# aaron-randreth/modulation-mfcc

Hardware: AMD Instinct MI355X
Metric: MFCC+mod-spectrum frames/sec (higher is better)
Workload: dtype f32; 1 GPU; BASELINE configs[2] per GPU: 1024 clips x 10 s x 16000 Hz, win 400 hop 160 n_fft 512, 40 mel (fmax 8000), 13 MFCC + modulation spectrum (rFFT 1024 over trajectories); frames_per_clip=1001, clips_total=1024, parallelism=clips sharded x1, hsa_ipc_mode_legacy=0, settle_calls=744, full=False, fused_tail=True

## Files before the change

### include/modmfcc.h

```cpp
#ifndef MODMFCC_H
#define MODMFCC_H

#include <stddef.h>
#include <stdint.h>

#ifdef __cplusplus
extern "C" {
#endif

#define MM_VERSION 123

typedef enum mm_status {
  MM_OK = 0,
  MM_ERR_INVALID_ARG = -1,
  MM_ERR_UNSUPPORTED = -2,
  MM_ERR_HIP = -3,
  MM_ERR_WORKSPACE = -4,
  MM_ERR_ALLOC = -5
} mm_status;

typedef struct mm_config {
  double sr;
  int32_t n_fft;
  int32_t win_length;
// ... 26 lines not shown
const char* mm_strerror(int status);
const char* mm_last_hip_error(void);

int mm_config_default(mm_config* cfg);
int mm_config_validate(const mm_config* cfg);
int64_t mm_num_frames(const mm_config* cfg, int64_t n_samples);
int32_t mm_num_bins(const mm_config* cfg);
int32_t mm_mod_fft_len(const mm_config* cfg, int64_t n_frames);
int mm_build_window(const mm_config* cfg, float* out );
int mm_build_mel(const mm_config* cfg, float* out );
int mm_build_dct(const mm_config* cfg, float* out );
int mm_build_mel_sweep(const mm_config* cfg, int n_waves, float* wlo ,
                       float* whi , int32_t* d , int32_t* part );
int mm_build_mel_runs(const mm_config* cfg, int n_waves, int32_t* hdr, int32_t hdr_cap, float* grp,
                      int32_t grp_cap, int32_t* part, int32_t* counts);
int mm_build_butter_sos(int order, double wn, double* sos );

int mm_plan_create(const mm_config* cfg, mm_plan** out);
int mm_plan_destroy(mm_plan* plan);
int mm_plan_config(const mm_plan* plan, mm_config* out);
int mm_plan_kernel_path(const mm_plan* plan);
int mm_plan_fused_dct(const mm_plan* plan);
int mm_plan_set_fuse_dct(mm_plan* plan, int on);
int mm_plan_fused_tail(const mm_plan* plan, int64_t batch, int64_t n_samples);
int mm_plan_set_fuse_tail(mm_plan* plan, int on);
int mm_plan_force_generic(mm_plan* plan, int on);
int mm_plan_set_variant(mm_plan* plan, int variant);
size_t mm_workspace_bytes(const mm_plan* plan, int64_t batch, int64_t n_samples);

int mm_mfcc_f32(mm_plan* plan, const float* d_audio, int64_t batch, int64_t n_samples,
                int64_t audio_stride, float* d_mfcc, void* d_workspace, size_t ws_bytes,
                void* stream);

int mm_logmel_f32(mm_plan* plan, const float* d_audio, int64_t batch, int64_t n_samples,
                  int64_t audio_stride, float* d_logmel, float* d_clipmax, void* stream);

int mm_stft_power_f32(mm_plan* plan, const float* d_audio, int64_t batch, int64_t n_samples,
                      int64_t audio_stride, float* d_power, void* stream);

int mm_rfft_f32(mm_plan* plan, const float* d_in, int64_t rows, int64_t in_len,
// ... 151 lines not shown
```

### modulation_mfcc_amd/_lib.py

```python
from __future__ import annotations

import ctypes as C
import os

_HERE = os.path.dirname(os.path.abspath(__file__))
LIB_PATH = os.environ.get("MODMFCC_LIB") or os.path.join(_HERE, "libmodmfcc.so")

MM_OK = 0
MM_ERR_INVALID_ARG = -1
MM_ERR_UNSUPPORTED = -2
MM_ERR_HIP = -3
MM_ERR_WORKSPACE = -4
MM_ERR_ALLOC = -5

STAGES = ("logmel", "dct", "modspec", "rfft", "power", "change", "init", "reserved")
MM_NUM_STAGES = 8


class mm_config(C.Structure):
    _fields_ = [
        ("sr", C.c_double),
        ("n_fft", C.c_int32),
        ("win_length", C.c_int32),
        ("hop_length", C.c_int32),
# ... 73 lines not shown

PROTOTYPES = {
    "mm_version": (C.c_int, []),
    "mm_strerror": (C.c_char_p, [C.c_int]),
    "mm_last_hip_error": (C.c_char_p, []),
    "mm_config_default": (C.c_int, [_cfgp]),
    "mm_config_validate": (C.c_int, [_cfgp]),
    "mm_num_frames": (_i64, [_cfgp, _i64]),
    "mm_num_bins": (C.c_int32, [_cfgp]),
    "mm_mod_fft_len": (C.c_int32, [_cfgp, _i64]),
    "mm_build_window": (C.c_int, [_cfgp, _vp]),
    "mm_build_mel": (C.c_int, [_cfgp, _vp]),
    "mm_build_dct": (C.c_int, [_cfgp, _vp]),
    "mm_build_mel_sweep": (C.c_int, [_cfgp, C.c_int, _vp, _vp, _vp, _vp]),
    "mm_build_mel_runs": (C.c_int, [_cfgp, C.c_int, _vp, C.c_int32, _vp, C.c_int32, _vp, _vp]),
    "mm_build_butter_sos": (C.c_int, [C.c_int, C.c_double, _vp]),
    "mm_plan_create": (C.c_int, [_cfgp, C.POINTER(_vp)]),
    "mm_plan_destroy": (C.c_int, [_vp]),
    "mm_plan_config": (C.c_int, [_vp, _cfgp]),
    "mm_plan_kernel_path": (C.c_int, [_vp]),
    "mm_plan_fused_dct": (C.c_int, [_vp]),
    "mm_plan_set_fuse_dct": (C.c_int, [_vp, C.c_int]),
    "mm_plan_fused_tail": (C.c_int, [_vp, _i64, _i64]),
    "mm_plan_set_fuse_tail": (C.c_int, [_vp, C.c_int]),
    "mm_mfcc_modspec_f32": (C.c_int, [_vp, _vp, _i64, _i64, _i64, _vp, _vp, _vp, C.c_size_t, _vp]),
    "mm_plan_force_generic": (C.c_int, [_vp, C.c_int]),
    "mm_plan_set_variant": (C.c_int, [_vp, C.c_int]),
    "mm_workspace_bytes": (C.c_size_t, [_vp, _i64, _i64]),
    "mm_mfcc_f32": (C.c_int, [_vp, _vp, _i64, _i64, _i64, _vp, _vp, C.c_size_t, _vp]),
    "mm_logmel_f32": (C.c_int, [_vp, _vp, _i64, _i64, _i64, _vp, _vp, _vp]),
    "mm_stft_power_f32": (C.c_int, [_vp, _vp, _i64, _i64, _i64, _vp, _vp]),
    "mm_rfft_f32": (C.c_int, [_vp, _vp, _i64, _i64, _i64, C.c_int32, _vp, _vp]),
    "mm_modspec_f32": (C.c_int, [_vp, _vp, _i64, _i64, _vp, _vp]),
    "mm_mfcc_change_f64": (C.c_int, [_vp, _vp, _i64, _i64, C.c_int32, C.c_int32, _vp, C.c_int32, _vp,
                                     C.c_int32, _vp, _vp, C.c_size_t, _vp]),
    "mm_sosfiltfilt_f64": (C.c_int, [_vp, _i64, _i64, _i64, _vp, C.c_int32, _vp, _vp, C.c_size_t, _vp]),
    "mm_sosfiltfilt_workspace_bytes": (C.c_size_t, [_i64, _i64]),
    "mm_sosfiltfilt_f32_f64": (C.c_int, [_vp, _i64, _i64, _i64, _vp, C.c_int32, _vp, _vp, C.c_size_t, _vp]),
    "mm_stencil_f64": (C.c_int, [C.POINTER(mm_stencil), _vp, _i64, _i64, _i64, _vp, _vp]),
# ... 75 lines not shown
```

### modulation_mfcc_amd/csrc/mm_api.hip

```cpp
#include <memory>
#include <utility>

#include "mm_common.h"
#include "mm_plan.h"

thread_local std::string g_hip_err;

struct StftParams {
  const float* audio;
  int64_t batch, n_samples, stride, n_frames;
  int n_fft, log2nc, hop, n_bins, n_mels;
  float preemph, amin, db_offset;
  const float* window;
  const float2* tw;
  const int* mel_start;
  const int* mel_len;
  const int* mel_off;
  const float* mel_w;
  float* out_power;
  float* out_logmel;
  int* clip_key;
  int frames_per_wave;
};

// ... 240 lines not shown
}
int mm_build_mel_sweep(const mm_config* c, int n_waves, float* wlo, float* whi, int32_t* d, int32_t* part) {
  int s = mm::validate(c);
  if (s) return s;
  if (n_waves < 1 || !wlo || !whi || !d || !part) return MM_ERR_INVALID_ARG;
  std::vector<float> mel((size_t)c->n_mels * (c->n_fft / 2 + 1));
  mm::build_mel(*c, mel.data());
  mm::MelSweep sw;
  if (!mm::build_mel_sweep(*c, mel.data(), n_waves, &sw)) return MM_ERR_UNSUPPORTED;
  std::memcpy(wlo, sw.wlo.data(), sw.wlo.size() * 4);
  std::memcpy(whi, sw.whi.data(), sw.whi.size() * 4);
  std::memcpy(d, sw.d.data(), sw.d.size() * 4);
  std::memcpy(part, sw.part.data(), sw.part.size() * 4);
  return MM_OK;
}
int mm_build_mel_runs(const mm_config* c, int n_waves, int32_t* hdr, int32_t hdr_cap, float* grp,
                      int32_t grp_cap, int32_t* part, int32_t* counts) {
  int s = mm::validate(c);
  if (s) return s;
  if (n_waves < 1 || !hdr || !grp || !part || !counts) return MM_ERR_INVALID_ARG;
  std::vector<float> mel((size_t)c->n_mels * (c->n_fft / 2 + 1));
  mm::build_mel(*c, mel.data());
  mm::MelSweep sw;
  if (!mm::build_mel_sweep(*c, mel.data(), n_waves, &sw)) return MM_ERR_UNSUPPORTED;
  mm::MelRuns r;
  mm::build_mel_runs(*c, sw, n_waves, &r);
  counts[0] = (int32_t)(r.hdr.size() / 4);
  counts[1] = (int32_t)(r.grp.size() / 8);
  if (counts[0] > hdr_cap || counts[1] > grp_cap) return MM_ERR_WORKSPACE;
  std::memcpy(hdr, r.hdr.data(), r.hdr.size() * 4);
  std::memcpy(grp, r.grp.data(), r.grp.size() * 4);
  std::memcpy(part, r.part.data(), r.part.size() * 4);
  return MM_OK;
}
int mm_build_butter_sos(int order, double wn, double* sos) { return mm::build_butter_sos(order, wn, sos); }


static std::vector<float> packed_run_table(const mm::MelRuns& r) {
  std::vector<float> tab(r.hdr.size() + r.grp.size());
  std::memcpy(tab.data(), r.hdr.data(), r.hdr.size() * 4);
  std::memcpy(tab.data() + r.hdr.size(), r.grp.data(), r.grp.size() * 4);
  for (size_t g = 0; g < r.grp.size() / 8; ++g) {
    float* q = tab.data() + r.hdr.size() + 8 * g;
    const float t[8] = {q[0], q[4], q[1], q[5], q[2], q[6], q[3], q[7]};
    std::memcpy(q, t, sizeof t);
  }
  return tab;
}
// ... 279 lines not shown
    const double wts_d[16] = {1, 1, 1, MM_S16F_W, 1, 1, 1, MM_S16F_W, 1, 1, 1, MM_S16F_W, 1, 1, 1, MM_S16F_W};
    double extra[16];
    for (int w = 0; w < 16; ++w) extra[w] = (!single && wts_d[w] < 1.0) ? 700.0 : 0.0;
    mm::MelSweep swf;
    if (!mm::build_mel_sweep(c, h.melp, 16, &swf, single ? nullptr : wts_d)) return;
    mm::MelRuns rf;
    mm::build_mel_runs(c, swf, 16, &rf);
    if (ef.skip)
      for (size_t r = 0; r < rf.hdr.size() / 4; ++r) {
        const int d = rf.hdr[4 * r + 3];
        if (d >= 0 && d < c.n_mels && ef.empty[d]) rf.hdr[4 * r + 0] |= 1 << 16;
      }
    const std::vector<float> tab = packed_run_table(rf);
    std::vector<int> wave_of_part;
    const std::vector<int> part = balance_parts_over_simds(rf, extra, &wave_of_part);
    unsigned long long roles = ~0ull;
    for (int f = 0; f < 4; ++f) {
      const int w = single ? f : wave_of_part[4 * f + 3];
      roles = (roles & ~(0xFull << (4 * w))) | ((unsigned long long)f << (4 * w));
    }
    const size_t tab_end = (size_t)MM_S16_TAB_OFF(p->s16.nr, xa) + tab.size() * 4;
    const unsigned lt_off = (unsigned)align_up(tab_end, 16);
    const unsigned dcta_off = lt_off + (single ? 1u : 2u) * (unsigned)lt_rows * 320u;
    const unsigned red_off = (unsigned)align_up((size_t)dcta_off + dcta.size() * 4, 16);
    const size_t lds = (size_t)red_off + 2 * 16 * 8;
    if (lds > MM_LM_LDS_MAX) continue;
    mm_plan::S16F& f = p->s16f;
    f.ok = p->upload(&f.d_tab, tab.data(), tab.size() * 4) == MM_OK &&
           p->upload(&f.d_part, part.data(), part.size() * 4) == MM_OK &&
           p->upload(&f.d_dcta, dcta.data(), dcta.size() * 4) == MM_OK;
    if (!f.ok) return;
    f.n_runs = (int)(rf.hdr.size() / 4); f.n_tab16 = (int)(tab.size() / 4);
    f.lt_rows = lt_rows; f.nk = nk; f.kb = kbn; f.roles = roles;
    f.flags = (single ? MM_S16F_SINGLE : 0) | (ef.skip ? MM_S16F_SKIP : 0);
    f.lt_off = lt_off; f.dcta_off = dcta_off; f.red_off = red_off; f.lds_bytes = lds;
    if (!xa && p->s16.xa) {
      p->s16.xa = false;
      p->s16.lds_bytes = (size_t)MM_S16_TAB_OFF(p->s16.nr, false) + tab16_bytes;
    }
    return;
  }
}

static void setup_m12(mm_plan* p, const PlanHost& h) {
  const mm_config& c = p->cfg;
  mm_plan::M12& m = p->m12;
  M12Tables mt;
  const int s_floats = (47 * c.hop_length + 512 + 255) & ~255;
  const int nr = (s_floats / 256 + 15) / 16;
  if (nr > 3 || !build_m12_tables(*h.ce, h.melp, h.dct.data(), &mt)) return;
// ... 273 lines not shown
}

int mm_plan_set_fuse_dct(mm_plan* p, int on) {
  if (!p) return MM_ERR_INVALID_ARG;
  const int prev = !p->user.no_fuse;
  p->user.no_fuse = on ? 0 : 1;
  return prev;
}

int mm_plan_set_fuse_tail(mm_plan* p, int on) {
  if (!p) return MM_ERR_INVALID_ARG;
  const int prev = p->user.no_fuse_tail ? 0 : (p->user.fuse_tail_wide ? 2 : 1);
  p->user.no_fuse_tail = on ? 0 : 1;
  p->user.fuse_tail_wide = on == 2 ? 1 : 0;
  return prev;
}

int mm_plan_set_variant(mm_plan* p, int variant) {
  if (!p || variant < 0 || variant > MM_K_H16 || variant == MM_K_ANY) return MM_ERR_INVALID_ARG;
  const int prev = p->user.variant;
  p->user.variant = variant;
  return prev;
}

int mm_plan_force_generic(mm_plan* p, int on) {
  if (!p) return MM_ERR_INVALID_ARG;
  int prev = p->user.force_generic;
  p->user.force_generic = on ? 1 : 0;
  return prev;
}
// ... 151 lines not shown
  if (q.n_tiles > 0x7FFFFFFF) return MM_ERR_INVALID_ARG;
  int64_t grid = q.n_tiles < p->num_cus ? q.n_tiles : p->num_cus;
  if (d.kernel == MM_K_W8) {
    hipLaunchKernelGGL(mode == 0 ? logmel512_kernel<0> : logmel512_kernel<1>, dim3((unsigned)grid), dim3(512), p->w8.lds_bytes, st, q);
    return MM_OK;
  }
  q.mel_tab = (const float4*)p->w16.d_tab; q.n_runs = p->w16.n_runs; q.n_tab16 = p->w16.n_tab16;
  q.wave_part = p->w16.d_part;
  if (d.kernel == MM_K_W16) {
    hipLaunchKernelGGL(mode == 0 ? logmel512w_kernel<0> : logmel512w_kernel<1>, dim3((unsigned)grid), dim3(1024), p->w16.lds_bytes, st, q);
    return MM_OK;
  }
  size_t lds = p->s16.lds_bytes;
  if (d.fused_dct) {
    const mm_plan::S16F& f = p->s16f;
    q.mel_tab = (const float4*)f.d_tab; q.n_runs = f.n_runs; q.n_tab16 = f.n_tab16;
    q.wave_part = f.d_part;
    q.out_mfcc = o.mfcc; q.key_nmin = o.key_nmin; q.dct_a = f.d_dcta; q.n_mfcc = p->cfg.n_mfcc;
    q.dct_nk = f.nk; q.dct_kb = f.kb; q.lt_rows = f.lt_rows;
    q.lt_off = f.lt_off; q.dcta_off = f.dcta_off; q.dct_roles = f.roles;
    q.dct_flags = f.flags | (p->s16.halfwin ? MM_S16F_HALFWIN : 0);
    q.lt_b2 = (f.flags & MM_S16F_SINGLE) ? 0 : f.lt_rows;
    if (p->cfg.top_db < 0.0f) q.out_logmel = nullptr;
    lds = f.lds_bytes;
    q.red_off = f.red_off;
    if (d.clip) {
      q.out_mod = (float2*)o.mod; q.n_mod = o.mod ? c.n_mod : 0; q.dct_t = p->base.d_dct_t; q.dct_kp = p->kp; q.top_db = p->cfg.top_db;
      grid = c.batch < p->num_cus ? c.batch : p->num_cus;
      const size_t per = (size_t)((c.batch + grid - 1) / grid);
      lds = std::max((size_t)f.red_off + per * 128, (size_t)MM_S16_FIN_TAB_OFF + MM_S16_FIN_TAB_BYTES);
      lds = std::max(lds, (size_t)MM_S16_DELTA_OFF((size_t)f.red_off, per, q.n_mod) + per * 4);
      if (q.n_mod == 2048) {
        q.tw = (const float2*)p->rf2k.d_lane_tab;
        lds = std::max(lds, (size_t)MM_S16_FIN2K_BYTES);
      }
      mode = 2;
// ... 258 lines not shown
```

### modulation_mfcc_amd/csrc/mm_fft16.hip.inc

```
#pragma once

namespace f16 {

__device__ __forceinline__ constexpr int P16(int k) { return 4 * (k & 3) + (k >> 2); }

__device__ __forceinline__ float2 cmulf(float2 a, float2 w) {
  return make_float2(fmaf(-a.y, w.y, a.x * w.x), fmaf(a.y, w.x, a.x * w.y));
}

__device__ __forceinline__ void radix4(float2& v0, float2& v1, float2& v2, float2& v3) {
  const float2 t0 = make_float2(v0.x + v2.x, v0.y + v2.y);
  const float2 t1 = make_float2(v0.x - v2.x, v0.y - v2.y);
  const float2 t2 = make_float2(v1.x + v3.x, v1.y + v3.y);
  const float2 t3 = make_float2(v1.x - v3.x, v1.y - v3.y);
  v0 = make_float2(t0.x + t2.x, t0.y + t2.y);
  v2 = make_float2(t0.x - t2.x, t0.y - t2.y);
  v1 = make_float2(t1.x + t3.y, t1.y - t3.x);
  v3 = make_float2(t1.x - t3.y, t1.y + t3.x);
}

__device__ __forceinline__ void dft16(float2 (&x)[16]) {
#pragma unroll
  for (int b = 0; b < 4; ++b) radix4(x[b], x[4 + b], x[8 + b], x[12 + b]);
  const float C1 = 0.92387953251128674f, S1 = 0.38268343236508977f, H = 0.70710678118654752f;
// ... 277 lines not shown
  const float* dct_a;
  int n_mfcc, dct_nk, dct_kb, lt_rows;
  int lt_b2;
  unsigned lt_off, dcta_off;
  unsigned long long dct_roles;
  int dct_flags;
  float2* out_mod;
  const float* dct_t;
  int n_mod, dct_kp;
  float top_db;
  unsigned red_off;
};

#define MM_S16F_SINGLE 1
#define MM_S16F_SKIP 2
#define MM_S16F_HALFWIN 8
#define MM_LM_PITCH 260
#define MM_LM_P_FLOATS (64 * MM_LM_PITCH)
#define MM_LM_EX_OFF (MM_LM_P_FLOATS * 4)
#define MM_LM_WIN_OFF (MM_LM_EX_OFF + 8 * f16::Geo<1>::WAVE_C * 8)
#define MM_LM_TAB_OFF (MM_LM_WIN_OFF + 512 * 4)

#include "mm_tile512.hip.inc"

struct LmItem {
  const float* a;
  int64_t t_first;
  bool live;
  bool interior;
};
// ... 143 lines not shown
```

### modulation_mfcc_amd/csrc/mm_internal.h

```cpp
#ifndef MM_INTERNAL_H
#define MM_INTERNAL_H

#include <vector>

#include "../../include/modmfcc.h"

namespace mm {

struct MelCsr {
  std::vector<int> start, len, off;
  std::vector<float> w;
};

struct MelSweep {
  std::vector<float> wlo, whi;
  std::vector<int> d;
  std::vector<int> part;
};
bool build_mel_sweep(const mm_config& c, const float* dense, int n_waves, MelSweep* out, const double* weights = nullptr);

struct MelRuns {
  std::vector<int> hdr;
  std::vector<float> grp;
  std::vector<int> part;
};
void build_mel_runs(const mm_config& c, const MelSweep& sw, int n_waves, MelRuns* out);

int validate(const mm_config* c);
void build_window(const mm_config& c, float* out);
void build_mel(const mm_config& c, float* out);
void build_dct(const mm_config& c, float* out);
void build_twiddles(int n, float* out);
int build_butter_sos(int order, double wn, double* sos);
void build_mel_csr(const mm_config& c, const float* dense, MelCsr* csr);

}
#endif
```

### modulation_mfcc_amd/csrc/mm_logmel16s.hip.inc

```
#pragma once

struct S16Fin {
  const float* logmel;
  float* mfcc;
  float2* mod;
  const float2* tw;
  const float* dct_t;
  int n_frames, n_mels, n_mfcc, dct_kp, n_mod;
  float top_db;
  float L0;
  const float* dct_e;
};

template <int R>
__device__ __forceinline__ void s16_fin_fill_tab(const float2* tw_generic, MM_LDS mm_v2f* tab) {
  typedef f16::Geo<R> G;
  const MM_GLOBAL mm_v2f* tw = (const MM_GLOBAL mm_v2f*)tw_generic;
  for (int idx = threadIdx.x; idx < G::LPR * MM_S16_FIN_REC + 15; idx += 1024) {
    mm_v2f v;
    if (idx < G::LPR * MM_S16_FIN_REC) {
      const int q = idx / MM_S16_FIN_REC, e = idx - q * MM_S16_FIN_REC;
      if (e < 15) {
        v = tw[(q * (e + 1)) * (MM_TW_N / G::NC)];
      } else {
// ... 383 lines not shown
  float* P = reinterpret_cast<float*>(smem);
  float* S = reinterpret_cast<float*>(smem + MM_S16_S_OFF(XA));
  const int lane = threadIdx.x & 63;
  const int wave = __builtin_amdgcn_readfirstlane(threadIdx.x >> 6);
  const int q = lane & 15, row = lane >> 4;
  const float* lt = reinterpret_cast<const float*>(smem + MM_S16_LT_OFF(NR, XA)) + q * MM_W16_LT_PITCH;

  for (int i = threadIdx.x; i < 16 * MM_W16_LT_PITCH; i += 1024)
    reinterpret_cast<float*>(smem + MM_S16_LT_OFF(NR, XA))[i] = p.lane_tab[i];
  if (threadIdx.x < 64 * 3) P[(threadIdx.x / 3) * MM_S16_PITCH(XA) + 257 + threadIdx.x % 3] = 0.0f;

  for (int i = threadIdx.x; i < p.n_tab16; i += 1024)
    reinterpret_cast<float4*>(smem + MM_S16_TAB_OFF(NR, XA))[i] = p.mel_tab[i];
  const int run0 = p.wave_part[wave * 4 + 0], run1 = p.wave_part[wave * 4 + 1];
  const int m0 = p.wave_part[wave * 4 + 2];
  const bool fused = MODE == 2 || (MODE == 1 && p.out_mfcc != nullptr);
  float* Lt = reinterpret_cast<float*>(smem + p.lt_off);
  const int role = fused ? (int)((p.dct_roles >> (4 * wave)) & 15) : 15;
  const bool lt_single = fused && p.lt_b2 == 0;
  const bool halfwin = NR <= 2 && (p.dct_flags & MM_S16F_HALFWIN) != 0;
  if (fused) {
    for (int i = threadIdx.x; i < (p.lt_b2 + p.lt_rows) * 80; i += 1024) Lt[i] = 0.0f;
    for (int i = threadIdx.x; i < p.dct_kb * p.dct_nk * 64 + 16 * p.dct_kb; i += 1024)
      reinterpret_cast<float*>(smem + p.dcta_off)[i] = p.dct_a[i];
  }
  float vmin = INFINITY;
  int pb = 0, pt0 = 0;
  bool has_prev = false;
  auto dct_tile = [&](const float* Lp, int cb, int ct0) {
    int ln = lane;
// ... 156 lines not shown
        v.z = (ok && s0 + 2 < n) ? v.z : 0.0f; v.w = (ok && s0 + 3 < n) ? v.w : 0.0f;
      } else {
        v.x = ok ? v.x : 0.0f; v.y = ok ? v.y : 0.0f; v.z = ok ? v.z : 0.0f; v.w = ok ? v.w : 0.0f;
      }
      reinterpret_cast<float4*>(S)[threadIdx.x + 1024 * j] = v;
    }
  };
  if (tile_begin < tile_end) {
    stage_load(b, tl);
    stage_store(tl);
  }
  __syncthreads();
  float2 wp[8];
  tile512_read_wp(wp, lt);

  MM_STAMP_BEGIN(16)
  for (int tile = tile_begin; tile < tile_end; ++tile) {
    const int t0 = tl * 64;
    MM_STAMP_AT(9)
    if (++ntl == tpc) { ntl = 0; ++nb; }
    const bool more = tile + 1 < tile_end;
    stage_load(more ? nb : b, more ? ntl : tl);
    MM_STAMP_AT(11)
    if (t0 + 4 * wave < (int)p.n_frames) {
    float2 x[16];
    if (halfwin) {
      if (hop_odd) {
#pragma unroll
        for (int n1 = 4; n1 < 12; ++n1) x[n1] = make_float2(sxf[32 * n1], sxf[32 * n1 + 1]);
      } else {
#pragma unroll
        for (int n1 = 4; n1 < 12; ++n1) x[n1] = sx[16 * n1];
      }
      const float4* w4 = reinterpret_cast<const float4*>(lt) + 2;
// ... 125 lines not shown
    if (MODE == 0) {
      tile512_store_power_tile(p.out_power, P, MM_S16_PITCH(XA), b, t0, p.n_frames, wave, 16, lane);
    } else {
      const bool valid = (t0 + lane) < p.n_frames;
      float* o = p.out_logmel + ((int64_t)b * p.n_mels + m0) * p.n_frames + t0 + lane;
      const float* pl = P + lane * MM_S16_PITCH(XA);
      const float4* hdr = reinterpret_cast<const float4*>(smem + MM_S16_TAB_OFF(NR, XA));
      const float4* grp = hdr + p.n_runs;
      float carry = 0.0f;
      if (run0 < run1) {
        float4 h = hdr[run0];
        for (int r = run0; r < run1; ++r) {
          const int k4e = __builtin_amdgcn_readfirstlane(__float_as_int(h.x));
          const int k4 = k4e & 0xFFFF;
          const bool empty_d = (k4e >> 16) & 1;
          const int ng = __builtin_amdgcn_readfirstlane(__float_as_int(h.y));
          const int go = __builtin_amdgcn_readfirstlane(__float_as_int(h.z));
          const int dd = __builtin_amdgcn_readfirstlane(__float_as_int(h.w));
          if (r + 1 < run1) h = hdr[r + 1];
          const float4* pp = reinterpret_cast<const float4*>(pl + k4);
          const MM_LDS mm_v4f* gw = (const MM_LDS mm_v4f*)(grp + 2 * go);
          asm volatile("" : "+v"(gw));
          float sa = 0.0f, sb = 0.0f;
          MM_STAMP_AT(12)
#pragma unroll 2
          for (int g = 0; g < ng; ++g) {
            const float4 pv = pp[g];
            const mm_v4f wa = gw[2 * g], wb = gw[2 * g + 1];
            sa = fmaf(wa.x, pv.x, sa); sb = fmaf(wa.y, pv.x, sb);
            sa = fmaf(wa.z, pv.y, sa); sb = fmaf(wa.w, pv.y, sb);
            sa = fmaf(wb.x, pv.z, sa); sb = fmaf(wb.y, pv.z, sb);
            sa = fmaf(wb.z, pv.w, sa); sb = fmaf(wb.w, pv.w, sb);
          }
          MM_STAMP_AT(13)
          float dbm = __builtin_nanf("");
          if (dd >= m0) {
            if (!empty_d) {
              const float v = carry + sa;
              const float db = 3.0102999566398120f * __builtin_amdgcn_logf(mm_max_raw_s(v, p.amin)) - p.db_offset;
              if (valid && p.out_logmel) *o = db;
              dbm = valid ? db : dbm;
              if (fused) Lt[((tile & 1) * p.lt_b2 + dd) * 80 + lane] = db;
            }
            o += p.n_frames;
          }
          mm_max_acc(vmax, dbm);
          mm_min_acc(vmin, dbm);
          carry = sb;
          MM_STAMP_AT(14)
        }
      }
      const bool clip_done = (tile + 1 == tile_end) || (ntl == 0);
      if (clip_done) {
        vmax = wave_max(vmax);
        if (p.key_nmin || clip_mode) vmin = wave_min(vmin);
        if (clip_mode) {
          if (lane == 0)
            reinterpret_cast<float2*>(smem + p.red_off)[(b - tile_begin / tpc) * 16 + wave] = make_float2(vmax, vmin);
        } else if (lane == 0 && vmax > -INFINITY) {
          atomicMax(p.clip_key + b, float_key(vmax));
          if (p.key_nmin) atomicMax(p.key_nmin + b, float_key(-vmin));
        }
        vmax = -INFINITY; vmin = INFINITY;
      }
    }
    MM_STAMP_AT(7)
    wg_barrier_lds();
    MM_STAMP_AT(8)
    pb = b; pt0 = t0; has_prev = true;
    b = nb; tl = ntl;
  }
  if (role < 4 && has_prev) dct_tile(Lt + (((tile_end - 1) & 1) * p.lt_b2) * 80, pb, pt0);
  if (clip_mode && has_prev) {
    S16Fin f;
    f.logmel = p.out_logmel; f.mfcc = p.out_mfcc; f.mod = p.out_mod; f.tw = p.tw; f.dct_t = p.dct_t;
    f.n_frames = (int)p.n_frames; f.n_mels = p.n_mels; f.n_mfcc = p.n_mfcc; f.dct_kp = p.dct_kp; f.n_mod = p.n_mod;
    f.top_db = p.top_db;
    f.dct_e = (p.dct_flags & MM_S16F_SKIP) ? p.dct_a + p.dct_kb * p.dct_nk * 64 : nullptr;
    f.L0 = mm_empty_level(p.amin, p.db_offset);
    s16_finalize_all(f, tile_begin / tpc, (tile_end - tile_begin) / tpc, p.red_off,
                     (int)((p.batch + gridDim.x - 1) / gridDim.x));
  }
  MM_STAMP_END(16)
}

// ... 34 lines not shown
```

### modulation_mfcc_amd/csrc/mm_plan.h

```cpp
#pragma once
#include "mm_common.h"

struct AnyPlan {
  int nn = 0, packed = 0, n_pass = 0, radix[16] = {0}, M = 0, log2M = 0, tpf = 64;
  unsigned grp_bytes = 0, b_off = 0, p_off = 0;
  float2 *d_tw = nullptr, *d_split = nullptr, *d_chirp = nullptr, *d_bhat = nullptr;
  float* d_tabpack = nullptr;
  int tab_floats = 0, o_tw = 0, o_split = 0, o_chirp = 0, o_melw = 0, o_mstart = 0, o_mlen = 0, o_moff = 0;
  bool lds_tab = false;
  bool ok = false;
  int fb = 0;
  int reg2 = 0, reg2_r2 = 0;
  unsigned fb_grp_bytes = 0;
};

#define MM_M12_MW 4
#define MM_M12_UMAX 12

#define MM_MAX_TIMED 16384
#define MM_MAX_SAMPLES (((int64_t)1 << 29) - 8192)

struct mm_plan {
  mm_config cfg{};
  int device = 0;
// ... 20 lines not shown
    int n_pairs = 0, n_tab16 = 0; size_t lds_bytes = 0;
  } h16;
  struct S16 {
    int nr = 0;
    bool xa = false;
    bool halfwin = false;
    size_t lds_bytes = 0;
  } s16;
  struct S16F {
    bool ok = false;
    float *d_tab = nullptr, *d_dcta = nullptr; int* d_part = nullptr;
    int n_runs = 0, n_tab16 = 0, lt_rows = 0, nk = 0, kb = 0;
    int flags = 0;
    unsigned lt_off = 0, dcta_off = 0, red_off = 0;
    unsigned long long roles = 0; size_t lds_bytes = 0;
  } s16f;
  struct M12 {
    bool ok = false, fused_dct = false;
    float *d_a = nullptr, *d_dct = nullptr, *d_zeros = nullptr;
    int units[MM_M12_MW * MM_M12_UMAX * 4] = {}, n_units[8] = {};
    int nb = 0, nr = 0, s_floats = 0, n_a2 = 0;
    unsigned win_off = 0, tw_off = 0, a_off = 0, dct_off = 0, part_off = 0, cnt_off = 0;
    size_t lds_bytes = 0;
  } m12;
  struct Wpf {
    bool ok = false; float *d_lane_tab = nullptr, *d_mel_lane = nullptr;
    int r = 0, waves = 0, group_max = 0; size_t lds_bytes = 0;
    bool w16 = false; size_t lds16 = 0;
    bool half = false; int pairs = 0;
    int waves_half = 0; size_t lds_half = 0;
// ... 1 lines not shown
  } wpf;
  struct DctFm {
    float* d_a = nullptr;
    float* d_wave_a = nullptr;
    int kb = 0, wave_nk = 0, ch = 0;
  } dctfm;
  struct Rf2k { bool ok = false; float* d_lane_tab = nullptr; } rf2k;
  AnyPlan any;

  struct Switches {
    int variant = 0;
    int force_generic = 0;
    int no_fuse = 0;
    int no_fuse_tail = 0;
    int fuse_tail_wide = 0;
  } user;
  struct Timing {
    int on = 0, ev_used = 0;
    std::vector<hipEvent_t> ev_pool;
    std::vector<int> ev_stage;
    double t_sum[MM_NUM_STAGES] = {};
    int64_t t_cnt[MM_NUM_STAGES] = {};
  } timing;

  mm_plan() = default;
  mm_plan(const mm_plan&) = delete; mm_plan& operator=(const mm_plan&) = delete;
  ~mm_plan() { for (void* d : owned) (void)hipFree(d); }
  template <class T>
  int upload(T** dst, const void* src, size_t bytes) {
    HIP_TRY(hipMalloc((void**)dst, bytes));
// ... 37 lines not shown
```

### modulation_mfcc_amd/csrc/mm_tables.cpp

```cpp
#include "mm_internal.h"

#include <algorithm>
#include <cmath>
#include <complex>
#include <cstring>
#include <vector>

namespace mm {

static const double kPi = 3.14159265358979323846;

int validate(const mm_config* c) {
  if (!c) return MM_ERR_INVALID_ARG;
  if (!(c->sr > 0.0)) return MM_ERR_INVALID_ARG;
  if (c->n_fft < 2) return MM_ERR_INVALID_ARG;
  if (c->n_fft > 8192) return MM_ERR_UNSUPPORTED;
  if (c->win_length < 1 || c->win_length > c->n_fft) return MM_ERR_INVALID_ARG;
  if (c->hop_length < 1) return MM_ERR_INVALID_ARG;
  if (c->n_mels < 1 || c->n_mels > 256) return MM_ERR_INVALID_ARG;
  if (c->n_mfcc < 1 || c->n_mfcc > c->n_mels) return MM_ERR_INVALID_ARG;
  if (!(c->fmin >= 0.0) || !(c->fmax > c->fmin)) return MM_ERR_INVALID_ARG;
  if (!(c->amin > 0.0f)) return MM_ERR_INVALID_ARG;
  if (c->center != 1) return MM_ERR_UNSUPPORTED;
  if (c->n_mod_fft != 0 &&
// ... 221 lines not shown
      const int left_waves = n_waves - 1 - w;
      if (n_mels - m1 < left_waves) m1 = std::max(m0, n_mels - left_waves);
    }
    int kb, ke;
    range_of(m0, m1, &kb, &ke);
    if (m1 <= m0) { kb = 0; ke = 0; }
    out->part[w * 4 + 0] = kb;
    out->part[w * 4 + 1] = ke;
    out->part[w * 4 + 2] = m0;
    out->part[w * 4 + 3] = m1;
    m = m1;
  }
  return true;
}

void build_mel_runs(const mm_config& c, const MelSweep& sw, int n_waves, MelRuns* out) {
  const int n_bins = c.n_fft / 2 + 1;
  out->hdr.clear(); out->grp.clear();
  out->part.assign((size_t)n_waves * 4, 0);
  for (int w = 0; w < n_waves; ++w) {
    const int m0 = sw.part[w * 4 + 2], m1 = sw.part[w * 4 + 3];
    out->part[w * 4 + 0] = (int)(out->hdr.size() / 4);
    out->part[w * 4 + 2] = m0;
    out->part[w * 4 + 3] = m1;
    if (m1 > m0) {
      for (int d = m0 - 1; d <= m1 - 1; ++d) {
        int ks = n_bins, ke = 0;
        for (int k = 0; k < n_bins; ++k)
          if (sw.d[k] == d && (sw.wlo[k] != 0.0f || sw.whi[k] != 0.0f)) { ks = std::min(ks, k); ke = std::max(ke, k + 1); }
        int g0 = 0, g1 = 0;
        if (ke > ks) { g0 = ks / 4; g1 = (ke + 3) / 4; }
        out->hdr.push_back(4 * g0);
        out->hdr.push_back(g1 - g0);
        out->hdr.push_back((int)(out->grp.size() / 8));
        out->hdr.push_back(d);
        for (int g = g0; g < g1; ++g) {
          float wl[4], wh[4];
          for (int u = 0; u < 4; ++u) {
            const int k = 4 * g + u;
            const bool in = (k >= ks && k < ke && k < n_bins && sw.d[k] == d);
            wl[u] = in ? sw.wlo[k] : 0.0f;
            wh[u] = in ? sw.whi[k] : 0.0f;
            if (d == m0 - 1) wl[u] = 0.0f;
            if (d == m1 - 1) wh[u] = 0.0f;
          }
          for (int u = 0; u < 4; ++u) out->grp.push_back(wl[u]);
          for (int u = 0; u < 4; ++u) out->grp.push_back(wh[u]);
        }
      }
    }
    out->part[w * 4 + 1] = (int)(out->hdr.size() / 4);
  }
}

}
```

### modulation_mfcc_amd/plan.py

```python
from __future__ import annotations

import ctypes as C
from dataclasses import dataclass, asdict

import numpy as np

from . import _lib


@dataclass(frozen=True)
class MfccConfig:
    sr: float = 10000.0
    n_fft: int = 512
    win_length: int = 250
    hop_length: int = 50
    n_mels: int = 128
    n_mfcc: int = 13
    fmin: float = 100.0
    fmax: float = 10000.0
    preemph: float = 0.0
    top_db: float = 80.0
    amin: float = 1e-10
    center: bool = True
    n_mod_fft: int = 0
# ... 63 lines not shown
                                                  d.ctypes.data, part.ctypes.data), "mm_build_mel_sweep")
        return wlo, whi, d, part

    def mel_runs(self, n_waves: int = 8):
        c = self.to_c()
        cap_r, cap_g = self.n_mels + 2 * n_waves + 8, self.n_bins // 4 + 2 * self.n_mels + 4 * n_waves + 8
        hdr = np.zeros((cap_r, 4), dtype=np.int32)
        grp = np.zeros((cap_g, 8), dtype=np.float32)
        part = np.zeros((n_waves, 4), dtype=np.int32)
        cnt = np.zeros(2, dtype=np.int32)
        _lib.check(_lib.load().mm_build_mel_runs(C.byref(c), n_waves, hdr.ctypes.data, cap_r,
                                                 grp.ctypes.data, cap_g, part.ctypes.data,
                                                 cnt.ctypes.data), "mm_build_mel_runs")
        return hdr[:cnt[0]], grp[:cnt[1]], part

    def asdict(self):
        return asdict(self)


def butter_sos(order: int, wn: float) -> np.ndarray:
    n_sec = (int(order) + 1) // 2
    out = np.empty((max(n_sec, 1), 6), dtype=np.float64)
    r = _lib.load().mm_build_butter_sos(int(order), float(wn), out.ctypes.data)
    if r < 0:
        _lib.check(int(r), "mm_build_butter_sos")
    return out[:r]


KERNEL_PATHS = ("generic", "radix16-w8", "radix16-w16", "radix16-wpf", "radix16-w16s", "radix16-m12", "any-length", "radix16-h32")

# ... 86 lines not shown
            v = 0
        elif isinstance(which, str):
            v = KERNEL_PATHS.index(which if which.startswith("radix16-") else "radix16-" + which)
        else:
            v = int(which)
        prev = self._lib.mm_plan_set_variant(self._h, v)
        if prev < 0:
            _lib.check(prev, "mm_plan_set_variant")
        return "auto" if prev == 0 else KERNEL_PATHS[prev]

    def fused_tail(self, batch, n_samples):
        return bool(self._lib.mm_plan_fused_tail(self._h, int(batch), int(n_samples)))

    def set_fuse_tail(self, on=True):
        return self._lib.mm_plan_set_fuse_tail(self._h, 2 if on == 2 else (1 if on else 0))

    def force_generic(self, on=True):
        return self._lib.mm_plan_force_generic(self._h, 1 if on else 0)

    def mfcc(self, audio, out=None):
        torch = _torch()
        audio = self._check_audio(audio)
        B, n = audio.shape
        T = self.cfg.num_frames(n)
        if out is None:
            out = torch.empty((B, self.cfg.n_mfcc, T), dtype=torch.float32, device=self.device)
        else:
            self._check_out(out, (B, self.cfg.n_mfcc, T), torch.float32, "mfcc")
        ws = self.workspace(B, n)
        with torch.cuda.device(self.device):
# ... 151 lines not shown
```

Baseline: 2.579 billion frames/s.

## Hand over boundary mel bands between waves via LDS instead of recomputing

Each wave in the fused logmel/DCT kernel used to recompute the mel band that straddles its partition boundary with its neighbour. The new run tables flag the first band as deferred and the last band as handed out. A wave writes its upper partial sum into LDS, and the next tile's finish step adds it to the neighbour's pending lower partial. This removes the duplicated boundary-band work, at the cost of moving the per-clip max/min reduction into a deferred step and adding a final barrier. It is enabled by default whenever the fused, non-single path has enough LDS rows.

Result: slower. 2.507 billion frames/s (-2.8%).

```diff
diff --git a/include/modmfcc.h b/include/modmfcc.h
--- a/include/modmfcc.h
+++ b/include/modmfcc.h
@@ -64,6 +64,8 @@
                        float* whi , int32_t* d , int32_t* part );
 int mm_build_mel_runs(const mm_config* cfg, int n_waves, int32_t* hdr, int32_t hdr_cap, float* grp,
                       int32_t grp_cap, int32_t* part, int32_t* counts);
+int mm_build_mel_runs_form(const mm_config* cfg, int n_waves, const double* weights, int handover, int32_t* hdr,
+                           int32_t hdr_cap, float* grp, int32_t grp_cap, int32_t* part, int32_t* counts);
 int mm_build_butter_sos(int order, double wn, double* sos );
 
 int mm_plan_create(const mm_config* cfg, mm_plan** out);
@@ -74,6 +76,8 @@
 int mm_plan_set_fuse_dct(mm_plan* plan, int on);
 int mm_plan_fused_tail(const mm_plan* plan, int64_t batch, int64_t n_samples);
 int mm_plan_set_fuse_tail(mm_plan* plan, int on);
+int mm_plan_mel_handover(const mm_plan* plan);
+int mm_plan_set_mel_handover(mm_plan* plan, int on);
 int mm_plan_force_generic(mm_plan* plan, int on);
 int mm_plan_set_variant(mm_plan* plan, int variant);
 size_t mm_workspace_bytes(const mm_plan* plan, int64_t batch, int64_t n_samples);
diff --git a/modulation_mfcc_amd/_lib.py b/modulation_mfcc_amd/_lib.py
--- a/modulation_mfcc_amd/_lib.py
+++ b/modulation_mfcc_amd/_lib.py
@@ -111,6 +111,7 @@
     "mm_build_dct": (C.c_int, [_cfgp, _vp]),
     "mm_build_mel_sweep": (C.c_int, [_cfgp, C.c_int, _vp, _vp, _vp, _vp]),
     "mm_build_mel_runs": (C.c_int, [_cfgp, C.c_int, _vp, C.c_int32, _vp, C.c_int32, _vp, _vp]),
+    "mm_build_mel_runs_form": (C.c_int, [_cfgp, C.c_int, _vp, C.c_int, _vp, C.c_int32, _vp, C.c_int32, _vp, _vp]),
     "mm_build_butter_sos": (C.c_int, [C.c_int, C.c_double, _vp]),
     "mm_plan_create": (C.c_int, [_cfgp, C.POINTER(_vp)]),
     "mm_plan_destroy": (C.c_int, [_vp]),
@@ -120,6 +121,8 @@
     "mm_plan_set_fuse_dct": (C.c_int, [_vp, C.c_int]),
     "mm_plan_fused_tail": (C.c_int, [_vp, _i64, _i64]),
     "mm_plan_set_fuse_tail": (C.c_int, [_vp, C.c_int]),
+    "mm_plan_mel_handover": (C.c_int, [_vp]),
+    "mm_plan_set_mel_handover": (C.c_int, [_vp, C.c_int]),
     "mm_mfcc_modspec_f32": (C.c_int, [_vp, _vp, _i64, _i64, _i64, _vp, _vp, _vp, C.c_size_t, _vp]),
     "mm_plan_force_generic": (C.c_int, [_vp, C.c_int]),
     "mm_plan_set_variant": (C.c_int, [_vp, C.c_int]),
diff --git a/modulation_mfcc_amd/csrc/mm_api.hip b/modulation_mfcc_amd/csrc/mm_api.hip
--- a/modulation_mfcc_amd/csrc/mm_api.hip
+++ b/modulation_mfcc_amd/csrc/mm_api.hip
@@ -278,17 +278,17 @@
   std::memcpy(part, sw.part.data(), sw.part.size() * 4);
   return MM_OK;
 }
-int mm_build_mel_runs(const mm_config* c, int n_waves, int32_t* hdr, int32_t hdr_cap, float* grp,
-                      int32_t grp_cap, int32_t* part, int32_t* counts) {
+static int mel_runs_out(const mm_config* c, int n_waves, const double* weights, bool handover, int32_t* hdr, int32_t hdr_cap,
+                        float* grp, int32_t grp_cap, int32_t* part, int32_t* counts) {
   int s = mm::validate(c);
   if (s) return s;
   if (n_waves < 1 || !hdr || !grp || !part || !counts) return MM_ERR_INVALID_ARG;
   std::vector<float> mel((size_t)c->n_mels * (c->n_fft / 2 + 1));
   mm::build_mel(*c, mel.data());
   mm::MelSweep sw;
-  if (!mm::build_mel_sweep(*c, mel.data(), n_waves, &sw)) return MM_ERR_UNSUPPORTED;
+  if (!mm::build_mel_sweep(*c, mel.data(), n_waves, &sw, weights)) return MM_ERR_UNSUPPORTED;
   mm::MelRuns r;
-  mm::build_mel_runs(*c, sw, n_waves, &r);
+  mm::build_mel_runs(*c, sw, n_waves, &r, handover);
   counts[0] = (int32_t)(r.hdr.size() / 4);
   counts[1] = (int32_t)(r.grp.size() / 8);
   if (counts[0] > hdr_cap || counts[1] > grp_cap) return MM_ERR_WORKSPACE;
@@ -296,6 +296,14 @@
   std::memcpy(grp, r.grp.data(), r.grp.size() * 4);
   std::memcpy(part, r.part.data(), r.part.size() * 4);
   return MM_OK;
+}
+int mm_build_mel_runs(const mm_config* c, int n_waves, int32_t* hdr, int32_t hdr_cap, float* grp,
+                      int32_t grp_cap, int32_t* part, int32_t* counts) {
+  return mel_runs_out(c, n_waves, nullptr, false, hdr, hdr_cap, grp, grp_cap, part, counts);
+}
+int mm_build_mel_runs_form(const mm_config* c, int n_waves, const double* weights, int handover, int32_t* hdr,
+                           int32_t hdr_cap, float* grp, int32_t grp_cap, int32_t* part, int32_t* counts) {
+  return mel_runs_out(c, n_waves, weights, handover != 0, hdr, hdr_cap, grp, grp_cap, part, counts);
 }
 int mm_build_butter_sos(int order, double wn, double* sos) { return mm::build_butter_sos(order, wn, sos); }
 
@@ -605,11 +613,14 @@
     const std::vector<float> tab = packed_run_table(rf);
     std::vector<int> wave_of_part;
     const std::vector<int> part = balance_parts_over_simds(rf, extra, &wave_of_part);
-    unsigned long long roles = ~0ull;
-    for (int f = 0; f < 4; ++f) {
-      const int w = single ? f : wave_of_part[4 * f + 3];
-      roles = (roles & ~(0xFull << (4 * w))) | ((unsigned long long)f << (4 * w));
-    }
+    auto roles_of = [&](const std::vector<int>& wop) {
+      unsigned long long roles = ~0ull;
+      for (int f = 0; f < 4; ++f) {
+        const int w = single ? f : wop[4 * f + 3];
+        roles = (roles & ~(0xFull << (4 * w))) | ((unsigned long long)f << (4 * w));
+      }
+      return roles;
+    };
     const size_t tab_end = (size_t)MM_S16_TAB_OFF(p->s16.nr, xa) + tab.size() * 4;
     const unsigned lt_off = (unsigned)align_up(tab_end, 16);
     const unsigned dcta_off = lt_off + (single ? 1u : 2u) * (unsigned)lt_rows * 320u;
@@ -622,9 +633,29 @@
            p->upload(&f.d_dcta, dcta.data(), dcta.size() * 4) == MM_OK;
     if (!f.ok) return;
     f.n_runs = (int)(rf.hdr.size() / 4); f.n_tab16 = (int)(tab.size() / 4);
-    f.lt_rows = lt_rows; f.nk = nk; f.kb = kbn; f.roles = roles;
+    f.lt_rows = lt_rows; f.nk = nk; f.kb = kbn; f.roles = roles_of(wave_of_part);
     f.flags = (single ? MM_S16F_SINGLE : 0) | (ef.skip ? MM_S16F_SKIP : 0);
     f.lt_off = lt_off; f.dcta_off = dcta_off; f.red_off = red_off; f.lds_bytes = lds;
+    if (!single && 4 * 16 <= 2 * lt_rows) {
+      mm::MelRuns rh;
+      mm::build_mel_runs(c, swf, 16, &rh, true);
+      for (size_t r = 0; r < rh.hdr.size() / 4; ++r) {
+        const int d = rh.hdr[4 * r + 3];
+        if (ef.skip && d >= 0 && d < c.n_mels && ef.empty[d]) rh.hdr[4 * r + 0] |= 1 << 16;
+      }
+      for (int w = 0; w < 16; ++w) {
+        const int m0 = rh.part[w * 4 + 2];
+        if (ef.skip && rh.part[w * 4 + 1] > rh.part[w * 4 + 0] && ef.empty[m0]) rh.part[w * 4 + 3] |= MM_RUN_PEND_EMPTY;
+      }
+      const std::vector<float> tab_h = packed_run_table(rh);
+      std::vector<int> wop_h;
+      const std::vector<int> part_h = balance_parts_over_simds(rh, extra, &wop_h);
+      if (p->upload(&f.d_tab_h, tab_h.data(), tab_h.size() * 4) == MM_OK &&
+          p->upload(&f.d_part_h, part_h.data(), part_h.size() * 4) == MM_OK) {
+        f.handover = true;
+        f.n_runs_h = (int)(rh.hdr.size() / 4); f.n_tab16_h = (int)(tab_h.size() / 4); f.roles_h = roles_of(wop_h);
+      }
+    }
     if (!xa && p->s16.xa) {
       p->s16.xa = false;
       p->s16.lds_bytes = (size_t)MM_S16_TAB_OFF(p->s16.nr, false) + tab16_bytes;
@@ -928,6 +959,18 @@
   p->user.no_fuse_tail = on ? 0 : 1;
   p->user.fuse_tail_wide = on == 2 ? 1 : 0;
   return prev;
+}
+
+int mm_plan_set_mel_handover(mm_plan* p, int on) {
+  if (!p) return MM_ERR_INVALID_ARG;
+  const int prev = !p->user.no_mel_handover;
+  p->user.no_mel_handover = on ? 0 : 1;
+  return prev;
+}
+
+int mm_plan_mel_handover(const mm_plan* p) {
+  if (!p) return MM_ERR_INVALID_ARG;
+  return p->s16f.ok && p->s16f.handover && !p->user.no_mel_handover ? 1 : 0;
 }
 
 int mm_plan_set_variant(mm_plan* p, int variant) {
@@ -1109,12 +1152,14 @@
   size_t lds = p->s16.lds_bytes;
   if (d.fused_dct) {
     const mm_plan::S16F& f = p->s16f;
-    q.mel_tab = (const float4*)f.d_tab; q.n_runs = f.n_runs; q.n_tab16 = f.n_tab16;
-    q.wave_part = f.d_part;
+    const bool handover = f.handover && !p->user.no_mel_handover;
+    q.mel_tab = (const float4*)(handover ? f.d_tab_h : f.d_tab);
+    q.n_runs = handover ? f.n_runs_h : f.n_runs; q.n_tab16 = handover ? f.n_tab16_h : f.n_tab16;
+    q.wave_part = handover ? f.d_part_h : f.d_part;
     q.out_mfcc = o.mfcc; q.key_nmin = o.key_nmin; q.dct_a = f.d_dcta; q.n_mfcc = p->cfg.n_mfcc;
     q.dct_nk = f.nk; q.dct_kb = f.kb; q.lt_rows = f.lt_rows;
-    q.lt_off = f.lt_off; q.dcta_off = f.dcta_off; q.dct_roles = f.roles;
-    q.dct_flags = f.flags | (p->s16.halfwin ? MM_S16F_HALFWIN : 0);
+    q.lt_off = f.lt_off; q.dcta_off = f.dcta_off; q.dct_roles = handover ? f.roles_h : f.roles;
+    q.dct_flags = f.flags | (p->s16.halfwin ? MM_S16F_HALFWIN : 0) | (handover ? MM_S16F_HANDOVER : 0);
     q.lt_b2 = (f.flags & MM_S16F_SINGLE) ? 0 : f.lt_rows;
     if (p->cfg.top_db < 0.0f) q.out_logmel = nullptr;
     lds = f.lds_bytes;
diff --git a/modulation_mfcc_amd/csrc/mm_fft16.hip.inc b/modulation_mfcc_amd/csrc/mm_fft16.hip.inc
--- a/modulation_mfcc_amd/csrc/mm_fft16.hip.inc
+++ b/modulation_mfcc_amd/csrc/mm_fft16.hip.inc
@@ -315,6 +315,7 @@
 
 #define MM_S16F_SINGLE 1
 #define MM_S16F_SKIP 2
+#define MM_S16F_HANDOVER 4
 #define MM_S16F_HALFWIN 8
 #define MM_LM_PITCH 260
 #define MM_LM_P_FLOATS (64 * MM_LM_PITCH)
diff --git a/modulation_mfcc_amd/csrc/mm_internal.h b/modulation_mfcc_amd/csrc/mm_internal.h
--- a/modulation_mfcc_amd/csrc/mm_internal.h
+++ b/modulation_mfcc_amd/csrc/mm_internal.h
@@ -24,7 +24,11 @@
   std::vector<float> grp;
   std::vector<int> part;
 };
-void build_mel_runs(const mm_config& c, const MelSweep& sw, int n_waves, MelRuns* out);
+void build_mel_runs(const mm_config& c, const MelSweep& sw, int n_waves, MelRuns* out, bool handover = false);
+#define MM_RUN_DEFER (1 << 17)
+#define MM_RUN_HANDOUT (1 << 18)
+#define MM_RUN_SLOTS(rd, wr) ((rd) | (wr) << 8)
+#define MM_RUN_PEND_EMPTY (1 << 16)
 
 int validate(const mm_config* c);
 void build_window(const mm_config& c, float* out);
diff --git a/modulation_mfcc_amd/csrc/mm_logmel16s.hip.inc b/modulation_mfcc_amd/csrc/mm_logmel16s.hip.inc
--- a/modulation_mfcc_amd/csrc/mm_logmel16s.hip.inc
+++ b/modulation_mfcc_amd/csrc/mm_logmel16s.hip.inc
@@ -421,6 +421,11 @@
     reinterpret_cast<float4*>(smem + MM_S16_TAB_OFF(NR, XA))[i] = p.mel_tab[i];
   const int run0 = p.wave_part[wave * 4 + 0], run1 = p.wave_part[wave * 4 + 1];
   const int m0 = p.wave_part[wave * 4 + 2];
+  const int slots = (MODE != 0 && (p.dct_flags & MM_S16F_HANDOVER)) ? p.wave_part[wave * 4 + 3] : 0xFFFF;
+  const bool has_pend = (slots & 0xFF) != 0xFF;
+  const bool pend_live = has_pend && !(slots & MM_RUN_PEND_EMPTY);
+  float pend = 0.0f;
+  bool prev_done = false;
   const bool fused = MODE == 2 || (MODE == 1 && p.out_mfcc != nullptr);
   float* Lt = reinterpret_cast<float*>(smem + p.lt_off);
   const int role = fused ? (int)((p.dct_roles >> (4 * wave)) & 15) : 15;
@@ -607,10 +612,38 @@
   float2 wp[8];
   tile512_read_wp(wp, lt);
 
+  auto finish_prev = [&](int par) {
+    if (pend_live) {
+      int ln = lane;
+      asm volatile("" : "+v"(ln));
+      const float v = Lt[(4 * (slots & 0xFF) + (ln >> 4)) * 80 + 64 + (ln & 15)] + pend;
+      const float db = 3.0102999566398120f * __builtin_amdgcn_logf(mm_max_raw_s(v, p.amin)) - p.db_offset;
+      const bool valid = (pt0 + ln) < p.n_frames;
+      if (valid && p.out_logmel) p.out_logmel[((int64_t)pb * p.n_mels + m0) * p.n_frames + pt0 + ln] = db;
+      if (fused) Lt[(par * p.lt_b2 + m0) * 80 + ln] = db;
+      const float dbm = valid ? db : __builtin_nanf("");
+      mm_max_acc(vmax, dbm);
+      mm_min_acc(vmin, dbm);
+    }
+    if (prev_done) {
+      vmax = wave_max(vmax);
+      if (p.key_nmin || clip_mode) vmin = wave_min(vmin);
+      if (clip_mode) {
+        if (lane == 0)
+          reinterpret_cast<float2*>(smem + p.red_off)[(pb - tile_begin / tpc) * 16 + wave] = make_float2(vmax, vmin);
+      } else if (lane == 0 && vmax > -INFINITY) {
+        atomicMax(p.clip_key + pb, float_key(vmax));
+        if (p.key_nmin) atomicMax(p.key_nmin + pb, float_key(-vmin));
+      }
+      vmax = -INFINITY; vmin = INFINITY;
+    }
+  };
+
   MM_STAMP_BEGIN(16)
   for (int tile = tile_begin; tile < tile_end; ++tile) {
     const int t0 = tl * 64;
     MM_STAMP_AT(9)
+    if (MODE != 0 && has_prev) finish_prev((tile & 1) ^ 1);
     if (++ntl == tpc) { ntl = 0; ++nb; }
     const bool more = tile + 1 < tile_end;
     stage_load(more ? nb : b, more ? ntl : tl);
@@ -766,6 +799,7 @@
           const int k4e = __builtin_amdgcn_readfirstlane(__float_as_int(h.x));
           const int k4 = k4e & 0xFFFF;
           const bool empty_d = (k4e >> 16) & 1;
+          const bool defer_d = (k4e & MM_RUN_DEFER) != 0, hand_d = (k4e & MM_RUN_HANDOUT) != 0;
           const int ng = __builtin_amdgcn_readfirstlane(__float_as_int(h.y));
           const int go = __builtin_amdgcn_readfirstlane(__float_as_int(h.z));
           const int dd = __builtin_amdgcn_readfirstlane(__float_as_int(h.w));
@@ -786,7 +820,10 @@
           }
           MM_STAMP_AT(13)
           float dbm = __builtin_nanf("");
-          if (dd >= m0) {
+          if (defer_d) {
+            pend = sa;
+            o += p.n_frames;
+          } else if (dd >= m0) {
             if (!empty_d) {
               const float v = carry + sa;
               const float db = 3.0102999566398120f * __builtin_amdgcn_logf(mm_max_raw_s(v, p.amin)) - p.db_offset;
@@ -799,28 +836,25 @@
           mm_max_acc(vmax, dbm);
           mm_min_acc(vmin, dbm);
           carry = sb;
+          if (hand_d) {
+            int ln = lane;
+            asm volatile("" : "+v"(ln));
+            Lt[(4 * (slots >> 8 & 0xFF) + (ln >> 4)) * 80 + 64 + (ln & 15)] = sb;
+          }
           MM_STAMP_AT(14)
         }
       }
-      const bool clip_done = (tile + 1 == tile_end) || (ntl == 0);
-      if (clip_done) {
-        vmax = wave_max(vmax);
-        if (p.key_nmin || clip_mode) vmin = wave_min(vmin);
-        if (clip_mode) {
-          if (lane == 0)
-            reinterpret_cast<float2*>(smem + p.red_off)[(b - tile_begin / tpc) * 16 + wave] = make_float2(vmax, vmin);
-        } else if (lane == 0 && vmax > -INFINITY) {
-          atomicMax(p.clip_key + b, float_key(vmax));
-          if (p.key_nmin) atomicMax(p.key_nmin + b, float_key(-vmin));
-        }
-        vmax = -INFINITY; vmin = INFINITY;
-      }
+      prev_done = (tile + 1 == tile_end) || (ntl == 0);
     }
     MM_STAMP_AT(7)
     wg_barrier_lds();
     MM_STAMP_AT(8)
     pb = b; pt0 = t0; has_prev = true;
     b = nb; tl = ntl;
+  }
+  if (MODE != 0 && has_prev) {
+    finish_prev((tile_end - 1) & 1);
+    if (p.dct_flags & MM_S16F_HANDOVER) wg_barrier_lds();
   }
   if (role < 4 && has_prev) dct_tile(Lt + (((tile_end - 1) & 1) * p.lt_b2) * 80, pb, pt0);
   if (clip_mode && has_prev) {
diff --git a/modulation_mfcc_amd/csrc/mm_plan.h b/modulation_mfcc_amd/csrc/mm_plan.h
--- a/modulation_mfcc_amd/csrc/mm_plan.h
+++ b/modulation_mfcc_amd/csrc/mm_plan.h
@@ -58,6 +58,8 @@
     int flags = 0;
     unsigned lt_off = 0, dcta_off = 0, red_off = 0;
     unsigned long long roles = 0; size_t lds_bytes = 0;
+    bool handover = false; float* d_tab_h = nullptr; int* d_part_h = nullptr;
+    int n_runs_h = 0, n_tab16_h = 0; unsigned long long roles_h = 0;
   } s16f;
   struct M12 {
     bool ok = false, fused_dct = false;
@@ -89,6 +91,7 @@
     int no_fuse = 0;
     int no_fuse_tail = 0;
     int fuse_tail_wide = 0;
+    int no_mel_handover = 0;
   } user;
   struct Timing {
     int on = 0, ev_used = 0;
diff --git a/modulation_mfcc_amd/csrc/mm_tables.cpp b/modulation_mfcc_amd/csrc/mm_tables.cpp
--- a/modulation_mfcc_amd/csrc/mm_tables.cpp
+++ b/modulation_mfcc_amd/csrc/mm_tables.cpp
@@ -259,23 +259,36 @@
   return true;
 }
 
-void build_mel_runs(const mm_config& c, const MelSweep& sw, int n_waves, MelRuns* out) {
+void build_mel_runs(const mm_config& c, const MelSweep& sw, int n_waves, MelRuns* out, bool handover) {
   const int n_bins = c.n_fft / 2 + 1;
   out->hdr.clear(); out->grp.clear();
   out->part.assign((size_t)n_waves * 4, 0);
+  std::vector<int> before(n_waves, -1), behind(n_waves, -1);
+  for (int w = 0, last = -1; w < n_waves; ++w)
+    if (sw.part[w * 4 + 3] > sw.part[w * 4 + 2]) {
+      before[w] = last;
+      if (last >= 0) behind[last] = w;
+      last = w;
+    }
   for (int w = 0; w < n_waves; ++w) {
     const int m0 = sw.part[w * 4 + 2], m1 = sw.part[w * 4 + 3];
     out->part[w * 4 + 0] = (int)(out->hdr.size() / 4);
     out->part[w * 4 + 2] = m0;
-    out->part[w * 4 + 3] = m1;
+    out->part[w * 4 + 3] = handover ? MM_RUN_SLOTS(0xFF, 0xFF) : m1;
     if (m1 > m0) {
-      for (int d = m0 - 1; d <= m1 - 1; ++d) {
+      const int d_first = handover && m0 > 0 ? m0 : m0 - 1;
+      if (handover)
+        out->part[w * 4 + 3] = MM_RUN_SLOTS(before[w] >= 0 ? w : 0xFF, behind[w] >= 0 ? behind[w] : 0xFF);
+      for (int d = d_first; d <= m1 - 1; ++d) {
         int ks = n_bins, ke = 0;
         for (int k = 0; k < n_bins; ++k)
           if (sw.d[k] == d && (sw.wlo[k] != 0.0f || sw.whi[k] != 0.0f)) { ks = std::min(ks, k); ke = std::max(ke, k + 1); }
         int g0 = 0, g1 = 0;
         if (ke > ks) { g0 = ks / 4; g1 = (ke + 3) / 4; }
-        out->hdr.push_back(4 * g0);
+        int flags = 0;
+        if (handover && d == m0 && before[w] >= 0) flags |= MM_RUN_DEFER;
+        if (handover && d == m1 - 1 && behind[w] >= 0) flags |= MM_RUN_HANDOUT;
+        out->hdr.push_back(4 * g0 | flags);
         out->hdr.push_back(g1 - g0);
         out->hdr.push_back((int)(out->grp.size() / 8));
         out->hdr.push_back(d);
@@ -286,8 +299,8 @@
             const bool in = (k >= ks && k < ke && k < n_bins && sw.d[k] == d);
             wl[u] = in ? sw.wlo[k] : 0.0f;
             wh[u] = in ? sw.whi[k] : 0.0f;
-            if (d == m0 - 1) wl[u] = 0.0f;
-            if (d == m1 - 1) wh[u] = 0.0f;
+            if (!handover && d == m0 - 1) wl[u] = 0.0f;
+            if (!handover && d == m1 - 1) wh[u] = 0.0f;
           }
           for (int u = 0; u < 4; ++u) out->grp.push_back(wl[u]);
           for (int u = 0; u < 4; ++u) out->grp.push_back(wh[u]);
diff --git a/modulation_mfcc_amd/plan.py b/modulation_mfcc_amd/plan.py
--- a/modulation_mfcc_amd/plan.py
+++ b/modulation_mfcc_amd/plan.py
@@ -101,6 +101,22 @@
                                                  cnt.ctypes.data), "mm_build_mel_runs")
         return hdr[:cnt[0]], grp[:cnt[1]], part
 
+    def mel_runs_handover(self, n_waves: int = 16, weights=None, handover: bool = True):
+        c = self.to_c()
+        cap_r, cap_g = self.n_mels + 2 * n_waves + 8, self.n_bins // 4 + 2 * self.n_mels + 4 * n_waves + 8
+        hdr = np.zeros((cap_r, 4), dtype=np.int32)
+        grp = np.zeros((cap_g, 8), dtype=np.float32)
+        part = np.zeros((n_waves, 4), dtype=np.int32)
+        cnt = np.zeros(2, dtype=np.int32)
+        w = None if weights is None else np.ascontiguousarray(weights, dtype=np.float64)
+        if w is not None and w.shape != (n_waves,):
+            raise ValueError("weights: one value per wave")
+        _lib.check(_lib.load().mm_build_mel_runs_form(C.byref(c), n_waves, None if w is None else w.ctypes.data,
+                                                      1 if handover else 0, hdr.ctypes.data, cap_r, grp.ctypes.data,
+                                                      cap_g, part.ctypes.data, cnt.ctypes.data),
+                   "mm_build_mel_runs_form")
+        return hdr[:cnt[0]], grp[:cnt[1]], part
+
     def asdict(self):
         return asdict(self)
 
@@ -217,6 +233,13 @@
 
     def set_fuse_tail(self, on=True):
         return self._lib.mm_plan_set_fuse_tail(self._h, 2 if on == 2 else (1 if on else 0))
+
+    @property
+    def mel_handover(self):
+        return bool(self._lib.mm_plan_mel_handover(self._h))
+
+    def set_mel_handover(self, on=True):
+        return bool(self._lib.mm_plan_set_mel_handover(self._h, 1 if on else 0))
 
     def force_generic(self, on=True):
         return self._lib.mm_plan_force_generic(self._h, 1 if on else 0)
```
